# hpcaitech/SkyComputing

Measured on AMD Instinct MI355X. Metric: sec_per_iter_bert160_mnli_bsz32, lower is better.
Workload: dtype bf16; 1 GPU; model=bert-160L-H1024-A16, global_batch=32, seq_len=128, parallelism=pp1, microbatches=1, schedule=gpipe, allocate=even, num_pipeline_layers=483, hipgraph=True

## Files before the change

skycomputing_amd/ops/build.py:

```python

from __future__ import annotations

import glob
import hashlib
import json
import os
import subprocess
import sys

HIP_DIR = os.path.join(os.path.dirname(os.path.abspath(__file__)), "hip")
LIB = os.path.join(HIP_DIR, "libskyhip.so")
STAMP = os.path.join(HIP_DIR, ".build_stamp.json")

HIPCC = os.environ.get("HIPCC", "hipcc")
ARCH = os.environ.get("SKY_GFX_ARCH", "gfx950")
CFLAGS = [
    f"--offload-arch={ARCH}", "-O3", "-std=c++17", "-fPIC",
    "-fvisibility=hidden", "-Wall", "-Wno-unused-function",
]


def _source_hash(sources: list[str]) -> str:
    h = hashlib.sha256()
    for s in sorted(sources) + sorted(glob.glob(os.path.join(HIP_DIR, "*.h"))):
        with open(s, "rb") as f:
            h.update(f.read())
    h.update(" ".join(CFLAGS).encode())
    return h.hexdigest()


def build(force: bool = False, verbose: bool = True) -> str:
    sources = sorted(glob.glob(os.path.join(HIP_DIR, "*.hip")))
    if not sources:
        raise RuntimeError(f"no .hip sources under {HIP_DIR}")
    want = _source_hash(sources)
    if not force and os.path.isfile(LIB) and os.path.isfile(STAMP):
        try:
            with open(STAMP) as f:
                if json.load(f).get("hash") == want:
                    if verbose:
                        print(f"[skyhip] up to date: {LIB}")
                    return LIB
        except Exception:
            pass
    objs = []
    for src in sources:
        obj = src.replace(".hip", ".o")
        cmd = [HIPCC, *CFLAGS, "-x", "hip", "-c", src, "-o", obj]
        if verbose:
            print("[skyhip]", " ".join(cmd))
        subprocess.run(cmd, check=True)
        objs.append(obj)
# ... 15 lines not shown
```

skycomputing_amd/ops/hip/attention_bwd.hip:

```cpp

#include "attn_common.h"

template <bool HAS_MASK, bool DBIAS>
__global__ __launch_bounds__(256, 3) void attn_bwd1s_kernel(
    const ushort_t* __restrict__ qkv, const ushort_t* __restrict__ dout,
    const ushort_t* __restrict__ mask, const float* __restrict__ m_io,
    const float* __restrict__ l_io, ushort_t* __restrict__ pdT,
    ushort_t* __restrict__ dsT, ushort_t* __restrict__ dqkv, int B, int S,
    int h, float scale, float keep, uint64_t salt,
    const unsigned long long* __restrict__ state, float* __restrict__ dbscr) {
  extern __shared__ __attribute__((aligned(16))) char lds[];
  const int tid = threadIdx.x;
  const int l = tid & 63;
  const int w = tid >> 6;
  const int lm = l & 15;
  const int lg = l >> 4;
  const int QB = (S + 63) / 64;
  const int bh = blockIdx.x / QB;
  const int qb = blockIdx.x % QB;
  const int b = bh / h;
  const int hh = bh % h;
  const int ts = 3 * h * ATT_D;
  const int NT = (S + 15) / 16;
  const uint64_t seed = rng_seed(salt, state);
// ... 46 lines not shown
    float mrow[4], lrow[4], dot[4];
    uint64_t zs[4][2];
#pragma unroll
    for (int r = 0; r < 4; ++r) {
      const int row = qtok_base + lg * 4 + r;
      const int rr = row < S ? row : S - 1;
      mrow[r] = m_io[(size_t)bh * S + rr];
      lrow[r] = 1.f / l_io[(size_t)bh * S + rr];
      dot[r] = 0.f;
      zs[r][0] = zs[r][1] = 0;
      if (keep < 1.f) att_drop_hash(zs[r], seed, bh, S, row, lm);
    }
#pragma unroll
    for (int r = 0; r < 4; ++r) {
      const int row = qtok_base + lg * 4 + r;
#pragma unroll
      for (int kt = 0; kt < 8; ++kt) {
        if (kt >= NT) continue;
        const int col = kt * 16 + lm;
        const float p = att_prob(sacc[kt][r], scale, mval[kt], mrow[r],
                                 lrow[r], row < S && col < S);
        float dp = dacc[kt][r];
        if (keep < 1.f) dp = att_drop_keep(zs[r], kt, keep16) ? dp * inv_keep : 0.f;
        dot[r] += dp * p;
      }
    }
#pragma unroll
    for (int r = 0; r < 4; ++r) dot[r] = row16_sum(dot[r]);
#pragma unroll
    for (int kt = 0; kt < 8; ++kt) {
      if (kt >= NT) continue;
      const int col = kt * 16 + lm;
      ushort4_t ds4, pd4;
#pragma unroll
      for (int r = 0; r < 4; ++r) {
        const int row = qtok_base + lg * 4 + r;
        const float p = att_prob(sacc[kt][r], scale, mval[kt], mrow[r],
                                 lrow[r], row < S && col < S);
        float pd = p, dp = dacc[kt][r];
        if (keep < 1.f) {
          const bool kbit = att_drop_keep(zs[r], kt, keep16);
          pd = kbit ? p * inv_keep : 0.f;
          dp = kbit ? dp * inv_keep : 0.f;
        }
        const float ds = scale * p * (dp - dot[r]);
        const int rl = lg * 4 + r;
        *(ushort_t*)lds_at(lds, swz(32768 + w * 4096 + rl * 256 + col * 2, rl, 15)) =
            f32_to_bf16(ds);
        ds4[r] = f32_to_bf16(ds);
        pd4[r] = f32_to_bf16(pd);
      }
      if (col < S) {
        const size_t o = ((size_t)bh * S + col) * S + qtok_base + lg * 4;
        if (qtok_base + lg * 4 + 3 < S) {
          *(ushort4_t*)(dsT + o) = ds4;
          *(ushort4_t*)(pdT + o) = pd4;
        } else {
#pragma unroll
          for (int r = 0; r < 4; ++r)
            if (qtok_base + lg * 4 + r < S) {
              dsT[o + r] = ds4[r];
              pdT[o + r] = pd4[r];
            }
        }
      }
    }
  }
  __syncthreads();

  float cs[4] = {0.f, 0.f, 0.f, 0.f};
  if (active) {
    f32x4 qacc[4];
    att_zero(qacc);
#pragma unroll
    for (int ks = 0; ks < 4; ++ks) {
      if (ks * 32 >= S) break;
      bf16x8 asr = *(const bf16x8*)lds_at(
          lds, swz(32768 + w * 4096 + lm * 256 + (ks * 32 + lg * 8) * 2, lm, 15));
#pragma unroll
      for (int ct = 0; ct < 4; ++ct) {
        bf16x8 bkt = abf_tr_rows64(lds, 16384, ks * 32 + lg * 8, ct * 4, lm);
        qacc[ct] = __builtin_amdgcn_mfma_f32_16x16x32_bf16(asr, bkt, qacc[ct], 0, 0, 0);
      }
// ... 390 lines not shown
```

skycomputing_amd/ops/hip/attn_common.h:

```cpp
#pragma once

#include "common.h"

typedef const __attribute__((address_space(1))) unsigned int* att_gas;
typedef __attribute__((address_space(3))) unsigned int* att_las;

typedef __attribute__((ext_vector_type(8))) short bf16x8;
typedef __attribute__((ext_vector_type(4))) float f32x4;

#define ATT_SMAX 128
#define ATT_D 64

DEV void* lds_at(char* base, int byte) { return (void*)(base + byte); }

DEV int swz(int byte_addr, int row, int rmask) {
  return byte_addr ^ ((row & rmask) << 4);
}

typedef __attribute__((ext_vector_type(4))) short s16x4_a;
typedef __attribute__((address_space(3))) s16x4_a* abf_las4;

DEV bf16x8 abf_tr_rows64(const char* lds_base, int off, int r0, int cq0,
                         int s4) {
  s16x4_a v[2];
// ... 78 lines not shown
    int gtok = tok0 + tok;
    if (clamp && gtok >= S) gtok = S - 1;
    const int c16s = (u & 7) ^ (tok & 7);
    __builtin_amdgcn_global_load_lds(
        (att_gas)(src + (size_t)gtok * tstride + c16s * 8),
        (att_las)lds_at(lds, off + u * 16), 16, 0, 0);
  }
}

DEV float att_prob(float s, float scale, float mv, float m, float inv_l,
                   bool valid) {
  float p = __expf(s * scale + mv - m) * inv_l;
  if (!valid) p = 0.f;
  return p;
}

DEV void att_drop_hash(uint64_t (&z)[2], uint64_t seed, int bh, int S,
                       int row, int lm) {
  const uint64_t base = ((uint64_t)bh * S + row) * 16 + lm;
  z[0] = rng_hash(seed, base * 2);
  z[1] = rng_hash(seed, base * 2 + 1);
}
DEV bool att_drop_keep(const uint64_t (&z)[2], int kt, unsigned keep16) {
  const uint64_t zz = kt < 4 ? z[0] : z[1];
  return (unsigned)((zz >> (16 * (kt & 3))) & 0xFFFFu) < keep16;
}

DEV void att_store_rows16(ushort_t* __restrict__ dst, int rstride,
                          const f32x4 (&acc)[4], int row0, int S, int lm,
                          int lg) {
#pragma unroll
  for (int ct = 0; ct < 4; ++ct) {
#pragma unroll
    for (int r = 0; r < 4; ++r) {
      const int row = row0 + lg * 4 + r;
      if (row < S) dst[(size_t)row * rstride + ct * 16 + lm] = f32_to_bf16(acc[ct][r]);
    }
  }
}

DEV void att_store_rows16x2(ushort_t* __restrict__ d0,
                            ushort_t* __restrict__ d1, int rstride,
                            const f32x4 (&a0)[4], const f32x4 (&a1)[4],
                            int row0, int S, int lm, int lg) {
#pragma unroll
  for (int ct = 0; ct < 4; ++ct) {
#pragma unroll
    for (int r = 0; r < 4; ++r) {
      const int row = row0 + lg * 4 + r;
      const int c = ct * 16 + lm;
      if (row < S) {
        d0[(size_t)row * rstride + c] = f32_to_bf16(a0[ct][r]);
        d1[(size_t)row * rstride + c] = f32_to_bf16(a1[ct][r]);
      }
    }
  }
}

DEV void att_colsum_rows16(float (&cs)[4], const f32x4 (&acc)[4], int row0,
                           int S, int lg) {
#pragma unroll
  for (int ct = 0; ct < 4; ++ct) {
#pragma unroll
    for (int r = 0; r < 4; ++r)
      if (row0 + lg * 4 + r < S) cs[ct] += bf16_to_f32(f32_to_bf16(acc[ct][r]));
  }
}

DEV void att_colsum_wave(float (&cs)[4]) {
#pragma unroll
  for (int ct = 0; ct < 4; ++ct) {
    cs[ct] += __shfl_xor(cs[ct], 16, 64);
    cs[ct] += __shfl_xor(cs[ct], 32, 64);
  }
}

#define ATT_LAUNCH_HM(has_mask, KERNEL, grid, lds_bytes, stream, ...)         \
  do {                                                                        \
    if (has_mask) {                                                           \
      constexpr bool HM = true;                                               \
      hipLaunchKernelGGL(KERNEL, grid, dim3(256), lds_bytes, stream,          \
                         __VA_ARGS__);                                        \
    } else {                                                                  \
      constexpr bool HM = false;                                              \
      hipLaunchKernelGGL(KERNEL, grid, dim3(256), lds_bytes, stream,          \
                         __VA_ARGS__);                                        \
// ... 3 lines not shown
```

skycomputing_amd/ops/hip/common.h:

```cpp
#pragma once

#include <hip/hip_runtime.h>
#include <hip/hip_bf16.h>
#include <stdint.h>
#include <type_traits>

#define WAVE 64
#define DEV __device__ __forceinline__

typedef unsigned short ushort_t;
typedef __attribute__((ext_vector_type(2))) unsigned short ushort2_t;
typedef __attribute__((ext_vector_type(4))) unsigned short ushort4_t;
typedef __attribute__((ext_vector_type(8))) unsigned short ushort8_t;
typedef __attribute__((ext_vector_type(4))) float float4_t;

DEV float bf16_to_f32(ushort_t u) {
  union { unsigned int i; float f; } v;
  v.i = ((unsigned int)u) << 16;
  return v.f;
}

DEV ushort_t f32_to_bf16(float f) {
  union { unsigned int i; float f; } v;
  v.f = f;
  unsigned int lsb = (v.i >> 16) & 1u;
  v.i += 0x7fffu + lsb;
  return (ushort_t)(v.i >> 16);
}

enum { DT_F32 = 0, DT_BF16 = 1 };

template <int DT> struct Vec8;
template <> struct Vec8<DT_BF16> {
  static DEV void load(const void* p, int64_t i8, float f[8]) {
    ushort8_t v = ((const ushort8_t*)p)[i8];
#pragma unroll
    for (int j = 0; j < 8; ++j) f[j] = bf16_to_f32(v[j]);
  }
  static DEV void store(void* p, int64_t i8, const float f[8]) {
    ushort8_t v;
#pragma unroll
    for (int j = 0; j < 8; ++j) v[j] = f32_to_bf16(f[j]);
    ((ushort8_t*)p)[i8] = v;
  }
};
template <> struct Vec8<DT_F32> {
  static DEV void load(const void* p, int64_t i8, float f[8]) {
    float4_t a = ((const float4_t*)p)[i8 * 2];
    float4_t b = ((const float4_t*)p)[i8 * 2 + 1];
#pragma unroll
    for (int j = 0; j < 4; ++j) { f[j] = a[j]; f[4 + j] = b[j]; }
  }
  static DEV void store(void* p, int64_t i8, const float f[8]) {
    float4_t a, b;
#pragma unroll
    for (int j = 0; j < 4; ++j) { a[j] = f[j]; b[j] = f[4 + j]; }
    ((float4_t*)p)[i8 * 2] = a;
    ((float4_t*)p)[i8 * 2 + 1] = b;
  }
};

template <int DT> DEV float load_elem(const void* p, int64_t i);
template <> DEV float load_elem<DT_F32>(const void* p, int64_t i) {
  return ((const float*)p)[i];
}
template <> DEV float load_elem<DT_BF16>(const void* p, int64_t i) {
  return bf16_to_f32(((const ushort_t*)p)[i]);
}
template <int DT> DEV void store_elem(void* p, int64_t i, float v);
template <> DEV void store_elem<DT_F32>(void* p, int64_t i, float v) {
  ((float*)p)[i] = v;
}
template <> DEV void store_elem<DT_BF16>(void* p, int64_t i, float v) {
  ((ushort_t*)p)[i] = f32_to_bf16(v);
}

// ... 35 lines not shown
}

DEV uint64_t rng_seed(uint64_t salt, const unsigned long long* state) {
  return salt + (state ? *state : 0ull) * 0xD1B54A32D192ED03ull;
}

DEV float rng_uniform(uint64_t seed, uint64_t idx) {
  return (float)(rng_hash(seed, idx) >> 40) * 0x1.0p-24f;
}

DEV bool rng_keep16(uint64_t seed, uint64_t idx, unsigned keep16) {
  uint64_t z = rng_hash(seed, idx >> 2);
  return (unsigned)((z >> (16 * (idx & 3))) & 0xFFFFu) < keep16;
}

#define RNG_DROP8(seed, i8, keep16, inv_keep, v, bits)                        \
  do {                                                                        \
    const uint64_t z0_ = rng_hash(seed, (uint64_t)(i8) * 2);                  \
    const uint64_t z1_ = rng_hash(seed, (uint64_t)(i8) * 2 + 1);              \
    bits = 0;                                                                 \
    _Pragma("unroll") for (int j_ = 0; j_ < 8; ++j_) {                        \
      const uint64_t zz_ = j_ < 4 ? z0_ : z1_;                                \
      const bool kb_ =                                                        \
          (unsigned)((zz_ >> (16 * (j_ & 3))) & 0xFFFFu) < (keep16);          \
      bits |= (unsigned)kb_ << j_;                                            \
      (v)[j_] = kb_ ? (v)[j_] * (inv_keep) : 0.f;                             \
    }                                                                         \
  } while (0)

DEV unsigned keep_to_16(float keep) {
  return keep >= 1.f ? 0x20000u : (unsigned)(keep * 65536.f + 0.5f);
}

DEV float erf_fast(float x) {
  const float ax = fabsf(x);
  const float t = 1.f / fmaf(0.3275911f, ax, 1.f);
  const float p = t * fmaf(t, fmaf(t, fmaf(t, fmaf(t, 1.061405429f, -1.453152027f),
                                           1.421413741f), -0.284496736f),
                           0.254829592f);
  const float r = 1.f - p * __expf(-ax * ax);
  return copysignf(r, x);
}
DEV float gelu_f(float x) { return 0.5f * x * (1.f + erf_fast(x * 0.70710678118654752f)); }
DEV float gelu_grad_f(float x) {
  const float k = 0.70710678118654752f;
  const float c = 0.3989422804014327f;
  float cdf = 0.5f * (1.f + erf_fast(x * k));
  float pdf = c * __expf(-0.5f * x * x);
  return cdf + x * pdf;
}

void sky_launch_colsum_final(hipStream_t s, const float* scratch, void* out,
                             int64_t cols, int64_t nslabs, int dtout);

struct SkyFinishJob {
  uint64_t scratch;
  uint64_t out[3];
  int64_t nslabs;
  int64_t cols;
  int32_t nv;
  int32_t dtout;
};
constexpr int SKY_FINISH_MAX_JOBS = 4;

static inline void sky_finish_job_set(SkyFinishJob* job, uint64_t scratch,
                                      uint64_t o0, uint64_t o1, uint64_t o2,
                                      int64_t nslabs, int64_t cols, int nv,
                                      int dtout) {
  *job = SkyFinishJob{scratch, {o0, o1, o2}, nslabs, cols, nv, dtout};
}

constexpr int MAX_SLABS = 1024;

template <int MAXCH = 8, class F>
static inline void dispatch_tags(int dt, bool has_res, bool drop, int ch,
                                 F&& f) {
  using std::integral_constant;
  auto by_ch = [&](auto DT, auto HR, auto DR) {
    if (ch <= 2) f(DT, HR, DR, integral_constant<int, 2>{});
    else if (ch <= 4) f(DT, HR, DR, integral_constant<int, 4>{});
    else if constexpr (MAXCH >= 8) f(DT, HR, DR, integral_constant<int, 8>{});
// ... 15 lines not shown
```

skycomputing_amd/ops/hip/elementwise.hip:

```cpp

#include "common.h"


template <int DT>
__global__ __launch_bounds__(256) void bias_gelu_fwd_vec_kernel(
    const void* __restrict__ x, const void* __restrict__ b,
    void* __restrict__ y, int64_t n8, int64_t cols8) {
  for (int64_t i8 = (int64_t)blockIdx.x * 256 + threadIdx.x; i8 < n8;
       i8 += (int64_t)gridDim.x * 256) {
    float v[8], bv[8];
    Vec8<DT>::load(x, i8, v);
    Vec8<DT>::load(b, i8 % cols8, bv);
#pragma unroll
    for (int j = 0; j < 8; ++j) v[j] = gelu_f(v[j] + bv[j]);
    Vec8<DT>::store(y, i8, v);
  }
}

template <int DT>
__global__ __launch_bounds__(256) void bias_gelu_fwd_kernel(
    const void* __restrict__ x, const void* __restrict__ b,
    void* __restrict__ y, int64_t n, int64_t cols) {
  for (int64_t i = (int64_t)blockIdx.x * 256 + threadIdx.x; i < n;
       i += (int64_t)gridDim.x * 256) {
// ... 74 lines not shown
  float bv[8];
  if (HAS_B) Vec8<DT>::load(b, c8, bv);
  float s[8] = {0.f};
  for (int64_t r = r0; r < r1; ++r) {
    float v[8], d[8];
    Vec8<DT>::load(x, r * cols8 + c8, v);
    Vec8<DT>::load(dy, r * cols8 + c8, d);
#pragma unroll
    for (int j = 0; j < 8; ++j) {
      d[j] *= gelu_grad_f(HAS_B ? v[j] + bv[j] : v[j]);
      s[j] += d[j];
    }
    Vec8<DT>::store(dx, r * cols8 + c8, d);
  }
#pragma unroll
  for (int j = 0; j < 8; ++j) scratch[(slab * cols8 + c8) * 8 + j] = s[j];
}

template <int DT, bool HAS_B>
__global__ __launch_bounds__(256) void bias_gelu_bwd_cs_kernel(
    const void* __restrict__ dy, const void* __restrict__ x,
    const void* __restrict__ b, void* __restrict__ dx,
    float* __restrict__ scratch, int64_t rows, int64_t cols8,
    int64_t rows_per_slab) {
  const int64_t nwin = cols8 >> 8;
  const int64_t win = blockIdx.x % nwin;
  const int64_t slab = blockIdx.x / nwin;
  const int64_t c8 = win * 256 + threadIdx.x;
  const int64_t r0 = slab * rows_per_slab;
  const int64_t r1 = min(rows, r0 + rows_per_slab);
  float bv[8];
  if (HAS_B) Vec8<DT>::load(b, c8, bv);
  float s[8] = {0.f};
  for (int64_t r = r0; r < r1; ++r) {
    float v[8], d[8];
    Vec8<DT>::load(x, r * cols8 + c8, v);
    Vec8<DT>::load(dy, r * cols8 + c8, d);
#pragma unroll
    for (int j = 0; j < 8; ++j) {
      d[j] *= gelu_grad_f(HAS_B ? v[j] + bv[j] : v[j]);
      s[j] += d[j];
    }
    Vec8<DT>::store(dx, r * cols8 + c8, d);
  }
#pragma unroll
  for (int j = 0; j < 8; ++j) scratch[(slab * cols8 + c8) * 8 + j] = s[j];
}

template <int DT, int BLOCK>
__global__ __launch_bounds__(BLOCK) void colsum_part_kernel(
    const void* __restrict__ src, float* __restrict__ scratch, int64_t rows,
    int64_t cols8, int64_t rows_per_slab) {
  const int64_t c8 = (int64_t)blockIdx.x * BLOCK + threadIdx.x;
  if (c8 >= cols8) return;
  const int64_t slab = blockIdx.y;
  const int64_t r0 = slab * rows_per_slab;
  const int64_t r1 = min(rows, r0 + rows_per_slab);
  float s[8] = {0.f};
  for (int64_t r = r0; r < r1; ++r) {
    float v[8];
    Vec8<DT>::load(src, r * cols8 + c8, v);
#pragma unroll
    for (int j = 0; j < 8; ++j) s[j] += v[j];
  }
#pragma unroll
  for (int j = 0; j < 8; ++j) scratch[(slab * cols8 + c8) * 8 + j] = s[j];
}

template <int BLOCK, int DTOUT>
__global__ __launch_bounds__(1024) void colsum_final_kernel(
    const float* __restrict__ scratch, void* __restrict__ out, int64_t cols,
    int64_t nslabs) {
  __shared__ float lds[64][17];
  const int c = threadIdx.x & 15;
  const int g = threadIdx.x >> 4;
  const int64_t col = (int64_t)blockIdx.x * 16 + c;
// ... 359 lines not shown
```

skycomputing_amd/ops/hip/gemm2.hip:

```cpp

#include "common.h"

typedef __attribute__((ext_vector_type(8))) short bf16x8;
typedef __attribute__((ext_vector_type(4))) float f32x4;

#define G2_BM 256
#define G2_BN 256
#define G2_BK 64
#define G2_BLOCK 512
#define G2_LDS (128 * 1024)

typedef const __attribute__((address_space(1))) unsigned int* g2_gas;
typedef __attribute__((address_space(3))) unsigned int* g2_las;

DEV void g2_glds16(const void* g, void* l) {
  __builtin_amdgcn_global_load_lds((g2_gas)g, (g2_las)l, 16, 0, 0);
}

DEV int g2_swz(int byte_addr, int row) { return byte_addr ^ ((row & 7) << 4); }

enum { G2_EPI_NONE = 0, G2_EPI_BIAS = 1, G2_EPI_BIAS_GELU = 2 };

enum { G2_DIRECT = 0, G2_KMAJOR = 1 };

// ... 214 lines not shown
  }

  if (SPLIT) {
    float* out = Wk + (size_t)g * M * N;
#pragma unroll
    for (int i = 0; i < 8; ++i) {
      const int m = m0 + wr * 128 + i * 16 + lg * 4;
#pragma unroll
      for (int j = 0; j < 4; ++j) {
        const int n = n0 + wc * 64 + j * 16 + lm;
#pragma unroll
        for (int r = 0; r < 4; ++r)
          __builtin_nontemporal_store(acc[i][j][r],
                                      out + (size_t)(m + r) * N + n);
      }
    }
    return;
  }

  float bv[4];
  if (EPI != G2_EPI_NONE) {
#pragma unroll
    for (int j = 0; j < 4; ++j) {
      const int n = n0 + wc * 64 + j * 16 + lm;
      bv[j] = bias ? bf16_to_f32(bias[n]) : 0.f;
    }
  }
#pragma unroll
  for (int i = 0; i < 8; ++i) {
#pragma unroll
    for (int r = 0; r < 4; ++r) {
      const int m = m0 + wr * 128 + i * 16 + lg * 4 + r;
#pragma unroll
      for (int j = 0; j < 4; ++j) {
        const int n = n0 + wc * 64 + j * 16 + lm;
        float v = acc[i][j][r];
        if (EPI != G2_EPI_NONE) v += bv[j];
        if (EPI == G2_EPI_BIAS_GELU) {
          if (STORE_Z) Z[(size_t)m * ldc + n] = f32_to_bf16(v);
          v = gelu_f(v);
        }
        C[(size_t)m * ldc + n] = f32_to_bf16(v);
      }
    }
  }
}

template <int EPI, bool STORE_Z>
__global__ __launch_bounds__(256) void gemm2_reduce_kernel(
    const float* __restrict__ Wk, ushort_t* __restrict__ C,
    const ushort_t* __restrict__ bias, ushort_t* __restrict__ Z, long MN,
    int N, int ldc, int gsu) {
  const long i4 = ((long)blockIdx.x * 256 + threadIdx.x) * 4;
  if (i4 >= MN) return;
  f32x4 s = *(const f32x4*)(Wk + i4);
  for (int g = 1; g < gsu; ++g) {
    f32x4 p = *(const f32x4*)(Wk + (size_t)g * MN + i4);
#pragma unroll
    for (int r = 0; r < 4; ++r) s[r] += p[r];
  }
  const int m = (int)(i4 / N), n = (int)(i4 % N);
  ushort4_t o, zo;
#pragma unroll
  for (int r = 0; r < 4; ++r) {
    float v = s[r];
    if (EPI != G2_EPI_NONE) v += bf16_to_f32(bias[n + r]);
    if (EPI == G2_EPI_BIAS_GELU) {
      if (STORE_Z) zo[r] = f32_to_bf16(v);
      v = gelu_f(v);
    }
    o[r] = f32_to_bf16(v);
  }
  *(ushort4_t*)(C + (size_t)m * ldc + n) = o;
  if (EPI == G2_EPI_BIAS_GELU && STORE_Z) *(ushort4_t*)(Z + (size_t)m * ldc + n) = zo;
}

static int g2_set_lds(const void* f) {
  static const void* done[32];
  static int ndone = 0;
  for (int i = 0; i < ndone; ++i)
    if (done[i] == f) return 0;
  hipError_t e = hipFuncSetAttribute(
      f, hipFuncAttributeMaxDynamicSharedMemorySize, G2_LDS);
  if (e != hipSuccess) return (int)e;
  if (ndone < 32) done[ndone++] = f;
  return 0;
}

SKY_EXPORT int sky_gemm2(uint64_t stream, uint64_t A, uint64_t B, uint64_t C,
                         uint64_t bias, uint64_t Z, uint64_t Wk, int64_t M,
                         int64_t N, int64_t K, int64_t lda, int64_t ldb,
                         int64_t ldc, int transA, int transB, int epi,
                         int gsu) {
  if (M % G2_BM || N % G2_BN || K % G2_BK) return (int)hipErrorInvalidValue;
  if (gsu > 1 && (K % (gsu * G2_BK) || !Wk)) return (int)hipErrorInvalidValue;
  if (lda % 8 || ldb % 8 || ldc % 8) return (int)hipErrorInvalidValue;
  hipStream_t s = (hipStream_t)stream;
  const long ntiles = (M / G2_BM) * (N / G2_BN);
  dim3 grid((unsigned)(ntiles * (gsu > 1 ? gsu : 1)));
  const bool split = gsu > 1;
  const bool sz = Z != 0;
  int rc = 0;
#define G2K(AM, BM, EP, SZ, SP)                                                \
  do {                                                                         \
    rc = g2_set_lds((const void*)&gemm2_kernel<AM, BM, EP, SZ, SP>);           \
// ... 50 lines not shown
```

skycomputing_amd/ops/hip/layernorm.hip:

```cpp

#include "common.h"

#define LN_MAXCH 8


template <int CTRL, int ROW_MASK>
DEV float dpp_add(float v) {
  const int t = __builtin_amdgcn_update_dpp(0, __float_as_int(v), CTRL,
                                            ROW_MASK, 0xf, true);
  return v + __int_as_float(t);
}
DEV float wave_sum_dpp(float v) {
  v = dpp_add<0x111, 0xf>(v);
  v = dpp_add<0x112, 0xf>(v);
  v = dpp_add<0x114, 0xf>(v);
  v = dpp_add<0x118, 0xf>(v);
  v = dpp_add<0x142, 0xa>(v);
  v = dpp_add<0x143, 0xc>(v);
  return __int_as_float(__builtin_amdgcn_readlane(__float_as_int(v), 63));
}

struct LnDrop {
  uint64_t seed;
  unsigned keep16;
// ... 129 lines not shown
                                 uint64_t w, uint64_t b, uint64_t y,
                                 uint64_t mean, uint64_t rstd, int64_t rows,
                                 int64_t cols, float eps, int dt, float keep,
                                 uint64_t salt, uint64_t state) {
  hipStream_t s = (hipStream_t)stream;
  bool has_res = res != 0;
  bool drop = keep < 1.f;
  if (drop && !ln_fast_ok(cols)) return (int)hipErrorInvalidValue;
  if (ln_fast_ok(cols)) {
    unsigned grid = (unsigned)((rows + 3) / 4);
    if (grid > 8192u) grid = 8192u;
    dispatch_tags(dt, has_res, drop, ln_chunks(cols),
                  [&](auto DT, auto HR, auto DR, auto CH) {
      hipLaunchKernelGGL((ln_fwd_vec_kernel<DT, HR, DR, CH>), dim3(grid),
                         dim3(256), 0, s, (const void*)x, (const void*)res,
                         (const void*)w, (const void*)b, (void*)y,
                         (float*)mean, (float*)rstd, rows, cols, eps, keep,
                         salt, (const unsigned long long*)state);
    });
  } else {
    dim3 grid((unsigned)(rows < 4096 ? rows : 4096));
    dispatch_tags(dt, has_res, false, 0, [&](auto DT, auto HR, auto, auto) {
      hipLaunchKernelGGL((ln_fwd_kernel<DT, 256, HR>), grid, dim3(256), 0, s,
                         (const void*)x, (const void*)res, (const void*)w,
                         (const void*)b, (void*)y, (float*)mean, (float*)rstd,
                         rows, cols, eps);
    });
  }
  LAUNCH_CHECK();
  return 0;
}


template <int DT, bool HAS_RES, bool DROP, int CH, int NS>
__global__ __launch_bounds__(256) void ln_bwd_dx_cs_kernel(
    const void* __restrict__ dy, const void* __restrict__ x,
    const void* __restrict__ res, const void* __restrict__ w,
    const float* __restrict__ mean, const float* __restrict__ rstd,
    void* __restrict__ dx, void* __restrict__ dres,
    float* __restrict__ scratch, int64_t rows, int64_t cols, float keep,
    uint64_t salt, const unsigned long long* __restrict__ state) {
  const int lane = threadIdx.x & (WAVE - 1);
  const int wid = threadIdx.x / WAVE;
  const int64_t cols8 = cols / 8;
  const LnDrop drop(DROP, keep, salt, state);
  float xh[CH][8], dxh[CH][8];
  float sw[NS ? CH : 1][8], sb[NS ? CH : 1][8], sx[NS == 3 ? CH : 1][8];
  if constexpr (NS > 0) {
#pragma unroll
    for (int c = 0; c < CH; ++c)
#pragma unroll
      for (int j = 0; j < 8; ++j) {
        sw[c][j] = 0.f;
        sb[c][j] = 0.f;
        if constexpr (NS == 3) sx[c][j] = 0.f;
      }
  }
  unsigned kbits[CH];
  for (int64_t row = (int64_t)blockIdx.x * 4 + wid; row < rows;
       row += (int64_t)gridDim.x * 4) {
    const int64_t base8 = row * cols8;
    const float mu = mean[row], rs = rstd[row];
    float s1 = 0.f, s2 = 0.f;
#pragma unroll
    for (int c = 0; c < CH; ++c) {
      const int64_t i8 = (int64_t)c * WAVE + lane;
      if (i8 < cols8) {
// ... 9 lines not shown
          s2 += dxh[c][j] * xh[c][j];
          if constexpr (NS > 0) {
            sw[c][j] += dyv[j] * xh[c][j];
            sb[c][j] += dyv[j];
          }
        }
      }
    }
    s1 = wave_sum(s1) / (float)cols;
    s2 = wave_sum(s2) / (float)cols;
#pragma unroll
    for (int c = 0; c < CH; ++c) {
      const int64_t i8 = (int64_t)c * WAVE + lane;
      if (i8 < cols8) {
        float o[8];
#pragma unroll
        for (int j = 0; j < 8; ++j)
          o[j] = rs * (dxh[c][j] - s1 - xh[c][j] * s2);
        if (DROP && dres != nullptr) Vec8<DT>::store(dres, base8 + i8, o);
        if (DROP) {
#pragma unroll
          for (int j = 0; j < 8; ++j)
            o[j] = ((kbits[c] >> j) & 1u) ? o[j] * drop.inv_keep : 0.f;
        }
        if constexpr (NS == 3) {
#pragma unroll
          for (int j = 0; j < 8; ++j)
            sx[c][j] += DT == DT_BF16 ? bf16_to_f32(f32_to_bf16(o[j])) : o[j];
        }
        Vec8<DT>::store(dx, base8 + i8, o);
      }
    }
  }
  if constexpr (NS > 0) {
    __shared__ float mrg[NS][CH * 512];
    for (int i = threadIdx.x; i < NS * CH * 512; i += 256)
      (&mrg[0][0])[i] = 0.f;
    __syncthreads();
    for (int k = 0; k < 4; ++k) {
      if (wid == k) {
#pragma unroll
        for (int c = 0; c < CH; ++c) {
          const int64_t i8 = (int64_t)c * WAVE + lane;
          if (i8 < cols8) {
#pragma unroll
            for (int j = 0; j < 8; ++j) {
              mrg[0][i8 * 8 + j] += sw[c][j];
              mrg[1][i8 * 8 + j] += sb[c][j];
              if constexpr (NS == 3) mrg[2][i8 * 8 + j] += sx[c][j];
            }
          }
        }
      }
      __syncthreads();
    }
    float* base = scratch + (int64_t)blockIdx.x * NS * cols8 * 8;
    for (int i = threadIdx.x; i < cols8 * 8; i += 256) {
      base[i] = mrg[0][i];
      base[cols8 * 8 + i] = mrg[1][i];
      if constexpr (NS == 3) base[2 * cols8 * 8 + i] = mrg[2][i];
    }
  }
}

template <int DT, bool HAS_RES, bool DROP, int BLOCK>
__global__ __launch_bounds__(BLOCK) void ln_bwd_wb_part_kernel(
    const void* __restrict__ dy, const void* __restrict__ x,
// ... 109 lines not shown
    s2 = block_sum<BLOCK>(s2, lds) / (float)cols;
    for (int64_t c = threadIdx.x; c < cols; c += BLOCK) {
      float xv = load_elem<DT>(x, base + c);
      if (HAS_RES) xv += load_elem<DT>(res, base + c);
      float xhat = (xv - mu) * rs;
      float dxhat = load_elem<DT>(dy, base + c) * load_elem<DT>(w, c);
      store_elem<DT>(dx, base + c, rs * (dxhat - s1 - xhat * s2));
    }
  }
}

#define LN_XSUM_MAXCH 4

struct LnBwdArgs {
  hipStream_t s;
  uint64_t dy, x, res, w, mean, rstd, dx, dres, scratch;
  int64_t rows, cols;
  int dt;
  float keep;
  uint64_t salt, state;
};

template <int NS>
static int64_t ln_bwd_dx_launch(const LnBwdArgs& a) {
  unsigned gmax = 8192;
  if (NS > 0) {
    gmax = 512;
    if (const char* e = getenv("SKY_LN_CS_GRID")) gmax = (unsigned)atoi(e);
    if (gmax > (unsigned)MAX_SLABS) gmax = MAX_SLABS;
    if (gmax < 1) gmax = 1;
  }
  unsigned grid = (unsigned)((a.rows + 3) / 4);
  if (grid > gmax) grid = gmax;
  dispatch_tags<NS == 3 ? LN_XSUM_MAXCH : LN_MAXCH>(
      a.dt, a.res != 0, a.keep < 1.f, ln_chunks(a.cols),
      [&](auto DT, auto HR, auto DR, auto CH) {
        hipLaunchKernelGGL((ln_bwd_dx_cs_kernel<DT, HR, DR, CH, NS>),
                           dim3(grid), dim3(256), 0, a.s, (const void*)a.dy,
                           (const void*)a.x, (const void*)a.res,
                           (const void*)a.w, (const float*)a.mean,
                           (const float*)a.rstd, (void*)a.dx, (void*)a.dres,
                           (float*)a.scratch, a.rows, a.cols, a.keep, a.salt,
                           (const unsigned long long*)a.state);
      });
  return (int64_t)grid;
}

template <int NV>
static void ln_bwd_wb_final_launch(const LnBwdArgs& a, uint64_t dw,
                                   uint64_t db, uint64_t dxsum,
                                   int64_t nslabs) {
  auto launch = [&](auto kern) {
    hipLaunchKernelGGL(kern, dim3((unsigned)((a.cols + 15) / 16)), dim3(1024),
                       0, a.s, (const float*)a.scratch, (void*)dw, (void*)db,
                       (void*)dxsum, a.cols, nslabs);
  };
  if (a.dt == DT_BF16) launch(ln_bwd_wb_final_kernel<256, DT_BF16, NV>);
  else launch(ln_bwd_wb_final_kernel<256, DT_F32, NV>);
}

template <int NS>
static int ln_bwd_cs_launch(const LnBwdArgs& a, uint64_t dw, uint64_t db,
                            uint64_t dxsum, SkyFinishJob* job = nullptr) {
  const int64_t nslabs = ln_bwd_dx_launch<NS>(a);
  if (job)
    sky_finish_job_set(job, a.scratch, dw, db, dxsum, nslabs, a.cols, NS,
                       a.dt);
  else
    ln_bwd_wb_final_launch<NS>(a, dw, db, dxsum, nslabs);
  LAUNCH_CHECK();
  return 0;
}

SKY_EXPORT int sky_layernorm_bwd(uint64_t stream, uint64_t dy, uint64_t x,
                                 uint64_t res, uint64_t w, uint64_t mean,
                                 uint64_t rstd, uint64_t dx, uint64_t dw,
// ... 104 lines not shown
```

skycomputing_amd/ops/hip/sgd.hip:

```cpp

#include "common.h"

struct SgdDesc {
  uint64_t p, g, m, mom;
  int64_t n;
  int64_t pad;
};

template <int DT>
DEV void nt_load8(const void* p, int64_t i8, float f[8]);
template <>
DEV void nt_load8<DT_BF16>(const void* p, int64_t i8, float f[8]) {
  ushort8_t v = __builtin_nontemporal_load((const ushort8_t*)p + i8);
#pragma unroll
  for (int j = 0; j < 8; ++j) f[j] = bf16_to_f32(v[j]);
}
template <>
DEV void nt_load8<DT_F32>(const void* p, int64_t i8, float f[8]) {
  float4_t a = __builtin_nontemporal_load((const float4_t*)p + i8 * 2);
  float4_t b = __builtin_nontemporal_load((const float4_t*)p + i8 * 2 + 1);
#pragma unroll
  for (int j = 0; j < 4; ++j) { f[j] = a[j]; f[4 + j] = b[j]; }
}
template <int DT>
DEV void nt_store8(void* p, int64_t i8, const float f[8]);
template <>
DEV void nt_store8<DT_BF16>(void* p, int64_t i8, const float f[8]) {
  ushort8_t v;
#pragma unroll
  for (int j = 0; j < 8; ++j) v[j] = f32_to_bf16(f[j]);
  __builtin_nontemporal_store(v, (ushort8_t*)p + i8);
}
template <>
DEV void nt_store8<DT_F32>(void* p, int64_t i8, const float f[8]) {
  float4_t a, b;
#pragma unroll
  for (int j = 0; j < 4; ++j) { a[j] = f[j]; b[j] = f[4 + j]; }
  __builtin_nontemporal_store(a, (float4_t*)p + i8 * 2);
  __builtin_nontemporal_store(b, (float4_t*)p + i8 * 2 + 1);
}

template <int DT, int BLOCK, bool MASTER, bool MOM, int UNROLL = 2,
          bool NT = true>
__global__ __launch_bounds__(BLOCK) void sgd_kernel(
    const SgdDesc* __restrict__ descs, float lr, float momentum, float wd) {
  const SgdDesc d = descs[blockIdx.x];
  void* p = (void*)d.p;
  const void* g = (const void*)d.g;
  float* master = (float*)d.m;
  float* mbuf = (float*)d.mom;
  const int64_t n8 = d.n / 8;
  for (int64_t i8 = threadIdx.x; i8 < n8; i8 += UNROLL * BLOCK) {
#pragma unroll
    for (int u = 0; u < UNROLL; ++u) {
      const int64_t k8 = i8 + u * BLOCK;
      if (k8 >= n8) break;
      float gv[8], pv[8];
      if (NT) {
        nt_load8<DT>(g, k8, gv);
        if (MASTER) nt_load8<DT_F32>(master, k8, pv);
        else nt_load8<DT>(p, k8, pv);
      } else {
        Vec8<DT>::load(g, k8, gv);
        if (MASTER) Vec8<DT_F32>::load(master, k8, pv);
// ... 89 lines not shown
```

skycomputing_amd/ops/hiplib.py:

```python

from __future__ import annotations

import ctypes
import os

_LIB = None
_LIB_PATH = os.path.join(os.path.dirname(os.path.abspath(__file__)), "hip", "libskyhip.so")
_TRIED = False

_SIGNATURES: dict[str, list] = {}

FINISH_MAX_JOBS = 4

u64 = ctypes.c_uint64
i64 = ctypes.c_int64
i32 = ctypes.c_int32
f32 = ctypes.c_float
f64 = ctypes.c_double


class FinishJob(ctypes.Structure):

    _fields_ = [
        ("scratch", u64), ("out", u64 * 3), ("nslabs", i64), ("cols", i64),
        ("nv", i32), ("dtout", i32),
    ]


def _register_signatures(lib):
    sigs = {
        "sky_layernorm_fwd": [u64, u64, u64, u64, u64, u64, u64, u64, i64, i64, f32, i32, f32, u64, u64],
        "sky_layernorm_bwd": [u64, u64, u64, u64, u64, u64, u64, u64, u64, u64, u64, i64, i64, i32, f32, u64, u64, u64],
        "sky_layernorm_bwd_xsum": [u64, u64, u64, u64, u64, u64, u64, u64, u64, u64, u64, i64, i64, i32, f32, u64, u64, u64, u64],
        "sky_layernorm_bwd_xsum_ok": [i64],
        "sky_bias_gelu_fwd": [u64, u64, u64, u64, i64, i64, i32],
        "sky_bias_gelu_bwd": [u64, u64, u64, u64, u64, u64, u64, i64, i64, i32],
        "sky_masked_softmax_fwd": [u64, u64, u64, u64, i64, i64, i64, i64, f32, f32, u64, i32],
        "sky_masked_softmax_bwd": [u64, u64, u64, u64, i64, i64, i64, i64, f32, f32, u64, i32],
        "sky_embedding_fwd": [u64] * 12 + [i64, i64, i64, f32, i32],
        "sky_embedding_bwd": [u64] * 16 + [i64, i64, i32],
        "sky_sgd_step": [u64, u64, i64, f32, f32, f32, i32, i32],
        "sky_adamw_tick": [u64, u64, f64, f64],
        "sky_gradnorm_partials": [u64, u64, i64, u64, i32],
        "sky_gradnorm_finish": [u64, u64, i64, u64, f32],
        "sky_adamw_step": [u64, u64, i64, u64, f64, f64, f32, f32, i32, i32],
        "sky_detect_mem": [u64, u64],
        "sky_dropout_fwd": [u64, u64, u64, i64, f32, u64, u64, i32],
        "sky_dropout_bwd": [u64, u64, u64, i64, f32, u64, u64, i32],
        "sky_rng_tick": [u64, u64],
        "sky_colsum": [u64, u64, u64, u64, i64, i64, i32, i32],
        "sky_hblt_wgrad_bgrad": [u64, u64, u64, u64, u64, i64, i64, i64, i32],
        "sky_hblt_wgrad": [u64, u64, u64, u64, i64, i64, i64, i32],
        "sky_hblt_linear_gelu_aux": [u64, u64, u64, u64, u64, u64, i64, i64, i64, i32, i32],
        "sky_mfma_probe": [u64, u64, u64, u64],
        "sky_glds_probe": [u64, u64, u64, i32],
        "sky_gemm": [u64, u64, u64, u64, u64, u64, i64, i64, i64, i64, i64, i64, i32, i32, i32, i32, i32],
        "sky_gemm2": [u64, u64, u64, u64, u64, u64, u64, i64, i64, i64, i64, i64, i64, i32, i32, i32, i32],
        "sky_pack3": [u64, u64, u64, u64, u64, i64, i64, i64, i64, i32],
        "sky_attn_fwd": [u64, u64, u64, u64, u64, u64, i64, i64, i64, i64, f32, f32, u64, u64],
        "sky_attn_probs": [u64, u64, u64, u64, u64, u64, u64, i64, i64, i64, i64, f32, f32, u64, u64],
        "sky_attn_flash_fwd": [u64, u64, u64, u64, u64, u64, i64, i64, i64, i64, f32, f32, u64, u64],
        "sky_attn_bwd": [u64] * 9 + [i64, i64, i64, i64, f32, f32, u64, u64],
        "sky_attn_bwd_dbias": [u64] * 9 + [i64, i64, i64, i64, f32, f32, u64, u64, u64, u64, i32],
        "sky_attn_bwd_dbias_parts": [u64] * 9 + [i64, i64, i64, i64, f32, f32, u64, u64, u64, u64, i32, u64],
        "sky_layernorm_bwd_parts": [u64, u64, u64, u64, u64, u64, u64, u64, u64, u64, u64, i64, i64, i32, f32, u64, u64, u64, u64, u64],
        "sky_bias_gelu_bwd_parts": [u64, u64, u64, u64, u64, u64, u64, i64, i64, i32, u64],
        "sky_colsum_finish": [u64, u64, i32],
        "sky_attn_bwd_fused": [u64] * 7 + [i64, i64, i64, i64, f32, f32, u64, u64],
    }
    for name, argtypes in sigs.items():
        if hasattr(lib, name):
            fn = getattr(lib, name)
            fn.argtypes = argtypes
            fn.restype = ctypes.c_int
    return sigs


def lib():
    global _LIB, _TRIED
    if _LIB is None and not _TRIED:
        _TRIED = True
        if os.path.isfile(_LIB_PATH):
            _LIB = ctypes.CDLL(_LIB_PATH)
            _register_signatures(_LIB)
    return _LIB


def available() -> bool:
# ... 23 lines not shown
```

Baseline: 0.1014 sec/iter.

## Use hardware bf16 pack conversions, fast GELU math, and parallel LN-backward merge

Replaces the software round-to-nearest-even bf16 conversion with compiler `__bf16` conversions, adding paired and quad packing helpers used in attention, GEMM epilogues, elementwise and SGD stores. The goal is to let gfx950's packed f32-to-bf16 conversion instructions cut ALU work in epilogues. GELU backward now shares one exp between the cdf and pdf terms and uses a hardware reciprocal approximation, which may shift accuracy slightly. LayerNorm backward gains a per-wave LDS partial-sum merge that replaces the zeroed shared merge buffer. The diff also unrolls the bias-GELU backward row loop by two, and adds a probe kernel that checks rounding equivalence plus an env hook for extra compiler flags.

```diff
diff --git a/skycomputing_amd/ops/build.py b/skycomputing_amd/ops/build.py
--- a/skycomputing_amd/ops/build.py
+++ b/skycomputing_amd/ops/build.py
@@ -5,6 +5,7 @@
 import hashlib
 import json
 import os
+import shlex
 import subprocess
 import sys
 
@@ -18,6 +19,7 @@
     f"--offload-arch={ARCH}", "-O3", "-std=c++17", "-fPIC",
     "-fvisibility=hidden", "-Wall", "-Wno-unused-function",
 ]
+CFLAGS += shlex.split(os.environ.get("SKY_HIPCC_FLAGS", ""))
 
 
 def _source_hash(sources: list[str]) -> str:
diff --git a/skycomputing_amd/ops/hip/attention_bwd.hip b/skycomputing_amd/ops/hip/attention_bwd.hip
--- a/skycomputing_amd/ops/hip/attention_bwd.hip
+++ b/skycomputing_amd/ops/hip/attention_bwd.hip
@@ -102,6 +102,7 @@
       if (kt >= NT) continue;
       const int col = kt * 16 + lm;
       ushort4_t ds4, pd4;
+      float dsf[4], pdf[4];
 #pragma unroll
       for (int r = 0; r < 4; ++r) {
         const int row = qtok_base + lg * 4 + r;
@@ -114,11 +115,16 @@
           dp = kbit ? dp * inv_keep : 0.f;
         }
         const float ds = scale * p * (dp - dot[r]);
+        dsf[r] = ds;
+        pdf[r] = pd;
+      }
+      ds4 = f32x4_to_bf16x4(dsf[0], dsf[1], dsf[2], dsf[3]);
+      pd4 = f32x4_to_bf16x4(pdf[0], pdf[1], pdf[2], pdf[3]);
+#pragma unroll
+      for (int r = 0; r < 4; ++r) {
         const int rl = lg * 4 + r;
         *(ushort_t*)lds_at(lds, swz(32768 + w * 4096 + rl * 256 + col * 2, rl, 15)) =
-            f32_to_bf16(ds);
-        ds4[r] = f32_to_bf16(ds);
-        pd4[r] = f32_to_bf16(pd);
+            ds4[r];
       }
       if (col < S) {
         const size_t o = ((size_t)bh * S + col) * S + qtok_base + lg * 4;
diff --git a/skycomputing_amd/ops/hip/attn_common.h b/skycomputing_amd/ops/hip/attn_common.h
--- a/skycomputing_amd/ops/hip/attn_common.h
+++ b/skycomputing_amd/ops/hip/attn_common.h
@@ -134,9 +134,12 @@
 #pragma unroll
   for (int ct = 0; ct < 4; ++ct) {
 #pragma unroll
-    for (int r = 0; r < 4; ++r) {
+    for (int r = 0; r < 4; r += 2) {
       const int row = row0 + lg * 4 + r;
-      if (row < S) dst[(size_t)row * rstride + ct * 16 + lm] = f32_to_bf16(acc[ct][r]);
+      const unsigned int v2 = f32x2_to_bf16x2(acc[ct][r], acc[ct][r + 1]);
+      if (row < S) dst[(size_t)row * rstride + ct * 16 + lm] = (ushort_t)v2;
+      if (row + 1 < S)
+        dst[(size_t)(row + 1) * rstride + ct * 16 + lm] = (ushort_t)(v2 >> 16);
     }
   }
 }
@@ -148,12 +151,18 @@
 #pragma unroll
   for (int ct = 0; ct < 4; ++ct) {
 #pragma unroll
-    for (int r = 0; r < 4; ++r) {
+    for (int r = 0; r < 4; r += 2) {
       const int row = row0 + lg * 4 + r;
       const int c = ct * 16 + lm;
+      const unsigned int v0 = f32x2_to_bf16x2(a0[ct][r], a0[ct][r + 1]);
+      const unsigned int v1 = f32x2_to_bf16x2(a1[ct][r], a1[ct][r + 1]);
       if (row < S) {
-        d0[(size_t)row * rstride + c] = f32_to_bf16(a0[ct][r]);
-        d1[(size_t)row * rstride + c] = f32_to_bf16(a1[ct][r]);
+        d0[(size_t)row * rstride + c] = (ushort_t)v0;
+        d1[(size_t)row * rstride + c] = (ushort_t)v1;
+      }
+      if (row + 1 < S) {
+        d0[(size_t)(row + 1) * rstride + c] = (ushort_t)(v0 >> 16);
+        d1[(size_t)(row + 1) * rstride + c] = (ushort_t)(v1 >> 16);
       }
     }
   }
diff --git a/skycomputing_amd/ops/hip/bf16_round_probe.hip b/skycomputing_amd/ops/hip/bf16_round_probe.hip
--- /dev/null
+++ b/skycomputing_amd/ops/hip/bf16_round_probe.hip
@@ -0,0 +1,55 @@
+
+#include "common.h"
+
+DEV ushort_t bf16_round_formula(unsigned int i) {
+  const unsigned int lsb = (i >> 16) & 1u;
+  i += 0x7fffu + lsb;
+  return (ushort_t)(i >> 16);
+}
+
+DEV bool bf16_is_nan(ushort_t b) { return (b & 0x7fffu) > 0x7f80u; }
+
+constexpr unsigned PROBE_BLOCKS = 4096;
+
+__global__ __launch_bounds__(256) void bf16_round_probe_kernel(
+    unsigned long long* __restrict__ counts) {
+  const unsigned int t = blockIdx.x * 256u + threadIdx.x;
+  unsigned int bad = 0, nan_lost = 0, seen = 0;
+  for (unsigned int k = 0; k < 4096u; ++k) {
+    const unsigned int i = t + (k << 20);
+    const float f = __builtin_bit_cast(float, i);
+    const float g = __builtin_bit_cast(float, i * 2654435761u + 0x3f800001u);
+    const ushort_t ref = bf16_round_formula(i);
+    const ushort_t sc = f32_to_bf16(f);
+    const ushort_t lo = (ushort_t)f32x2_to_bf16x2(f, g);
+    const ushort_t hi = (ushort_t)(f32x2_to_bf16x2(g, f) >> 16);
+    if ((i & 0x7fffffffu) > 0x7f800000u) {
+      if (!bf16_is_nan(sc) || !bf16_is_nan(lo) || !bf16_is_nan(hi)) ++nan_lost;
+    } else {
+      if (sc != ref || lo != ref || hi != ref) ++bad;
+    }
+    ++seen;
+  }
+  for (int off = 32; off > 0; off >>= 1) {
+    bad += __shfl_xor(bad, off, 64);
+    nan_lost += __shfl_xor(nan_lost, off, 64);
+    seen += __shfl_xor(seen, off, 64);
+  }
+  if ((threadIdx.x & (WAVE - 1)) == 0) {
+    if (bad) atomicAdd(&counts[0], (unsigned long long)bad);
+    if (nan_lost) atomicAdd(&counts[1], (unsigned long long)nan_lost);
+    atomicAdd(&counts[2], (unsigned long long)seen);
+  }
+}
+
+SKY_EXPORT int sky_probe_bf16_round(uint64_t stream, uint64_t counts) {
+  if (counts == 0) return (int)hipErrorInvalidValue;
+  hipStream_t s = (hipStream_t)stream;
+  hipError_t e =
+      hipMemsetAsync((void*)counts, 0, 3 * sizeof(unsigned long long), s);
+  if (e != hipSuccess) return (int)e;
+  hipLaunchKernelGGL(bf16_round_probe_kernel, dim3(PROBE_BLOCKS), dim3(256), 0,
+                     s, (unsigned long long*)counts);
+  LAUNCH_CHECK();
+  return 0;
+}
diff --git a/skycomputing_amd/ops/hip/common.h b/skycomputing_amd/ops/hip/common.h
--- a/skycomputing_amd/ops/hip/common.h
+++ b/skycomputing_amd/ops/hip/common.h
@@ -20,12 +20,24 @@
   return v.f;
 }
 
+typedef __attribute__((ext_vector_type(2))) float float2_t;
+typedef __attribute__((ext_vector_type(2))) __bf16 bf16x2_t;
+typedef __attribute__((ext_vector_type(2))) unsigned int uint2_t;
+typedef __attribute__((ext_vector_type(4))) unsigned int uint4_t;
+
 DEV ushort_t f32_to_bf16(float f) {
-  union { unsigned int i; float f; } v;
-  v.f = f;
-  unsigned int lsb = (v.i >> 16) & 1u;
-  v.i += 0x7fffu + lsb;
-  return (ushort_t)(v.i >> 16);
+  return __builtin_bit_cast(ushort_t, (__bf16)f);
+}
+
+DEV unsigned int f32x2_to_bf16x2(float lo, float hi) {
+  const float2_t v = {lo, hi};
+  return __builtin_bit_cast(unsigned int,
+                            __builtin_convertvector(v, bf16x2_t));
+}
+
+DEV ushort4_t f32x4_to_bf16x4(float a, float b, float c, float d) {
+  const uint2_t v = {f32x2_to_bf16x2(a, b), f32x2_to_bf16x2(c, d)};
+  return __builtin_bit_cast(ushort4_t, v);
 }
 
 enum { DT_F32 = 0, DT_BF16 = 1 };
@@ -38,10 +50,10 @@
     for (int j = 0; j < 8; ++j) f[j] = bf16_to_f32(v[j]);
   }
   static DEV void store(void* p, int64_t i8, const float f[8]) {
-    ushort8_t v;
-#pragma unroll
-    for (int j = 0; j < 8; ++j) v[j] = f32_to_bf16(f[j]);
-    ((ushort8_t*)p)[i8] = v;
+    uint4_t v;
+#pragma unroll
+    for (int j = 0; j < 4; ++j) v[j] = f32x2_to_bf16x2(f[2 * j], f[2 * j + 1]);
+    ((uint4_t*)p)[i8] = v;
   }
 };
 template <> struct Vec8<DT_F32> {
@@ -143,21 +155,36 @@
   return keep >= 1.f ? 0x20000u : (unsigned)(keep * 65536.f + 0.5f);
 }
 
-DEV float erf_fast(float x) {
+
+DEV float erf_fast_e(float x, float e) {
   const float ax = fabsf(x);
+#ifdef SKY_GELU_IEEE_MATH
   const float t = 1.f / fmaf(0.3275911f, ax, 1.f);
+#else
+  const float t = __builtin_amdgcn_rcpf(fmaf(0.3275911f, ax, 1.f));
+#endif
   const float p = t * fmaf(t, fmaf(t, fmaf(t, fmaf(t, 1.061405429f, -1.453152027f),
                                            1.421413741f), -0.284496736f),
                            0.254829592f);
-  const float r = 1.f - p * __expf(-ax * ax);
+  const float r = 1.f - p * e;
   return copysignf(r, x);
+}
+DEV float erf_fast(float x) {
+  const float ax = fabsf(x);
+  return erf_fast_e(x, __expf(-ax * ax));
 }
 DEV float gelu_f(float x) { return 0.5f * x * (1.f + erf_fast(x * 0.70710678118654752f)); }
 DEV float gelu_grad_f(float x) {
   const float k = 0.70710678118654752f;
   const float c = 0.3989422804014327f;
+#ifdef SKY_GELU_IEEE_MATH
   float cdf = 0.5f * (1.f + erf_fast(x * k));
   float pdf = c * __expf(-0.5f * x * x);
+#else
+  const float e = __expf(-0.5f * x * x);
+  float cdf = 0.5f * (1.f + erf_fast_e(x * k, e));
+  float pdf = c * e;
+#endif
   return cdf + x * pdf;
 }
 
diff --git a/skycomputing_amd/ops/hip/elementwise.hip b/skycomputing_amd/ops/hip/elementwise.hip
--- a/skycomputing_amd/ops/hip/elementwise.hip
+++ b/skycomputing_amd/ops/hip/elementwise.hip
@@ -130,16 +130,29 @@
   float bv[8];
   if (HAS_B) Vec8<DT>::load(b, c8, bv);
   float s[8] = {0.f};
-  for (int64_t r = r0; r < r1; ++r) {
-    float v[8], d[8];
-    Vec8<DT>::load(x, r * cols8 + c8, v);
-    Vec8<DT>::load(dy, r * cols8 + c8, d);
+  auto row = [&](int64_t r, const float (&v)[8], float (&d)[8]) {
 #pragma unroll
     for (int j = 0; j < 8; ++j) {
       d[j] *= gelu_grad_f(HAS_B ? v[j] + bv[j] : v[j]);
       s[j] += d[j];
     }
     Vec8<DT>::store(dx, r * cols8 + c8, d);
+  };
+  int64_t r = r0;
+  for (; r + 1 < r1; r += 2) {
+    float va[8], da[8], vb[8], db[8];
+    Vec8<DT>::load(x, r * cols8 + c8, va);
+    Vec8<DT>::load(dy, r * cols8 + c8, da);
+    Vec8<DT>::load(x, (r + 1) * cols8 + c8, vb);
+    Vec8<DT>::load(dy, (r + 1) * cols8 + c8, db);
+    row(r, va, da);
+    row(r + 1, vb, db);
+  }
+  if (r < r1) {
+    float v[8], d[8];
+    Vec8<DT>::load(x, r * cols8 + c8, v);
+    Vec8<DT>::load(dy, r * cols8 + c8, d);
+    row(r, v, d);
   }
 #pragma unroll
   for (int j = 0; j < 8; ++j) scratch[(slab * cols8 + c8) * 8 + j] = s[j];
diff --git a/skycomputing_amd/ops/hip/gemm2.hip b/skycomputing_amd/ops/hip/gemm2.hip
--- a/skycomputing_amd/ops/hip/gemm2.hip
+++ b/skycomputing_amd/ops/hip/gemm2.hip
@@ -270,15 +270,22 @@
     for (int r = 0; r < 4; ++r) {
       const int m = m0 + wr * 128 + i * 16 + lg * 4 + r;
 #pragma unroll
-      for (int j = 0; j < 4; ++j) {
+      for (int j = 0; j < 4; j += 2) {
         const int n = n0 + wc * 64 + j * 16 + lm;
-        float v = acc[i][j][r];
-        if (EPI != G2_EPI_NONE) v += bv[j];
+        float v0 = acc[i][j][r], v1 = acc[i][j + 1][r];
+        if (EPI != G2_EPI_NONE) { v0 += bv[j]; v1 += bv[j + 1]; }
         if (EPI == G2_EPI_BIAS_GELU) {
-          if (STORE_Z) Z[(size_t)m * ldc + n] = f32_to_bf16(v);
-          v = gelu_f(v);
+          if (STORE_Z) {
+            const unsigned int z2 = f32x2_to_bf16x2(v0, v1);
+            Z[(size_t)m * ldc + n] = (ushort_t)z2;
+            Z[(size_t)m * ldc + n + 16] = (ushort_t)(z2 >> 16);
+          }
+          v0 = gelu_f(v0);
+          v1 = gelu_f(v1);
         }
-        C[(size_t)m * ldc + n] = f32_to_bf16(v);
+        const unsigned int c2 = f32x2_to_bf16x2(v0, v1);
+        C[(size_t)m * ldc + n] = (ushort_t)c2;
+        C[(size_t)m * ldc + n + 16] = (ushort_t)(c2 >> 16);
       }
     }
   }
@@ -298,17 +305,19 @@
     for (int r = 0; r < 4; ++r) s[r] += p[r];
   }
   const int m = (int)(i4 / N), n = (int)(i4 % N);
+  float v[4];
   ushort4_t o, zo;
 #pragma unroll
   for (int r = 0; r < 4; ++r) {
-    float v = s[r];
-    if (EPI != G2_EPI_NONE) v += bf16_to_f32(bias[n + r]);
-    if (EPI == G2_EPI_BIAS_GELU) {
-      if (STORE_Z) zo[r] = f32_to_bf16(v);
-      v = gelu_f(v);
-    }
-    o[r] = f32_to_bf16(v);
-  }
+    v[r] = s[r];
+    if (EPI != G2_EPI_NONE) v[r] += bf16_to_f32(bias[n + r]);
+  }
+  if (EPI == G2_EPI_BIAS_GELU) {
+    if (STORE_Z) zo = f32x4_to_bf16x4(v[0], v[1], v[2], v[3]);
+#pragma unroll
+    for (int r = 0; r < 4; ++r) v[r] = gelu_f(v[r]);
+  }
+  o = f32x4_to_bf16x4(v[0], v[1], v[2], v[3]);
   *(ushort4_t*)(C + (size_t)m * ldc + n) = o;
   if (EPI == G2_EPI_BIAS_GELU && STORE_Z) *(ushort4_t*)(Z + (size_t)m * ldc + n) = zo;
 }
diff --git a/skycomputing_amd/ops/hip/layernorm.hip b/skycomputing_amd/ops/hip/layernorm.hip
--- a/skycomputing_amd/ops/hip/layernorm.hip
+++ b/skycomputing_amd/ops/hip/layernorm.hip
@@ -185,7 +185,8 @@
 }
 
 
-template <int DT, bool HAS_RES, bool DROP, int CH, int NS>
+#define LN_PMERGE_OK(DROP, CH, NS) ((CH) <= 2 && (NS) > 0 && (DROP))
+template <int DT, bool HAS_RES, bool DROP, int CH, int NS, bool PMERGE = false>
 __global__ __launch_bounds__(256) void ln_bwd_dx_cs_kernel(
     const void* __restrict__ dy, const void* __restrict__ x,
     const void* __restrict__ res, const void* __restrict__ w,
@@ -261,7 +262,46 @@
       }
     }
   }
-  if constexpr (NS > 0) {
+  if constexpr (NS > 0 && PMERGE) {
+    static_assert(LN_PMERGE_OK(DROP, CH, NS), "see LN_PMERGE_OK");
+    __shared__ __attribute__((aligned(16))) float part[4][NS][CH * 512];
+#pragma unroll
+    for (int c = 0; c < CH; ++c)
+#pragma unroll
+      for (int j = 0; j < 8; ++j) {
+        asm volatile("" : "+v"(sw[c][j]), "+v"(sb[c][j]));
+        if constexpr (NS == 3) asm volatile("" : "+v"(sx[c][j]));
+      }
+#pragma unroll
+    for (int c = 0; c < CH; ++c) {
+      const int64_t i8 = (int64_t)c * WAVE + lane;
+      if (i8 < cols8) {
+        float4_t* pw = (float4_t*)&part[wid][0][i8 * 8];
+        float4_t* pb = (float4_t*)&part[wid][1][i8 * 8];
+        pw[0] = float4_t{sw[c][0], sw[c][1], sw[c][2], sw[c][3]};
+        pw[1] = float4_t{sw[c][4], sw[c][5], sw[c][6], sw[c][7]};
+        pb[0] = float4_t{sb[c][0], sb[c][1], sb[c][2], sb[c][3]};
+        pb[1] = float4_t{sb[c][4], sb[c][5], sb[c][6], sb[c][7]};
+        if constexpr (NS == 3) {
+          float4_t* px = (float4_t*)&part[wid][2][i8 * 8];
+          px[0] = float4_t{sx[c][0], sx[c][1], sx[c][2], sx[c][3]};
+          px[1] = float4_t{sx[c][4], sx[c][5], sx[c][6], sx[c][7]};
+        }
+      }
+    }
+    __syncthreads();
+    float* base = scratch + (int64_t)blockIdx.x * NS * cols8 * 8;
+    const int n4 = (int)(cols8 * 2);
+    for (int i4 = threadIdx.x; i4 < n4; i4 += 256) {
+#pragma unroll
+      for (int v = 0; v < NS; ++v) {
+        float4_t a = {0.f, 0.f, 0.f, 0.f};
+#pragma unroll
+        for (int k = 0; k < 4; ++k) a += *(const float4_t*)&part[k][v][i4 * 4];
+        *(float4_t*)(base + (int64_t)v * cols8 * 8 + (int64_t)i4 * 4) = a;
+      }
+    }
+  } else if constexpr (NS > 0) {
     __shared__ float mrg[NS][CH * 512];
     for (int i = threadIdx.x; i < NS * CH * 512; i += 256)
       (&mrg[0][0])[i] = 0.f;
@@ -437,16 +477,28 @@
   }
   unsigned grid = (unsigned)((a.rows + 3) / 4);
   if (grid > gmax) grid = gmax;
+  [[maybe_unused]] const bool serial =
+      NS > 0 &&
+      (getenv("SKY_LN_MERGE_SERIAL") != nullptr || (a.scratch & 15) != 0);
   dispatch_tags<NS == 3 ? LN_XSUM_MAXCH : LN_MAXCH>(
       a.dt, a.res != 0, a.keep < 1.f, ln_chunks(a.cols),
       [&](auto DT, auto HR, auto DR, auto CH) {
-        hipLaunchKernelGGL((ln_bwd_dx_cs_kernel<DT, HR, DR, CH, NS>),
-                           dim3(grid), dim3(256), 0, a.s, (const void*)a.dy,
-                           (const void*)a.x, (const void*)a.res,
-                           (const void*)a.w, (const float*)a.mean,
-                           (const float*)a.rstd, (void*)a.dx, (void*)a.dres,
-                           (float*)a.scratch, a.rows, a.cols, a.keep, a.salt,
-                           (const unsigned long long*)a.state);
+        auto launch = [&](auto kern) {
+          hipLaunchKernelGGL(kern, dim3(grid), dim3(256), 0, a.s,
+                             (const void*)a.dy, (const void*)a.x,
+                             (const void*)a.res, (const void*)a.w,
+                             (const float*)a.mean, (const float*)a.rstd,
+                             (void*)a.dx, (void*)a.dres, (float*)a.scratch,
+                             a.rows, a.cols, a.keep, a.salt,
+                             (const unsigned long long*)a.state);
+        };
+        if constexpr (LN_PMERGE_OK(DR, CH, NS)) {
+          if (!serial) {
+            launch(ln_bwd_dx_cs_kernel<DT, HR, DR, CH, NS, true>);
+            return;
+          }
+        }
+        launch(ln_bwd_dx_cs_kernel<DT, HR, DR, CH, NS, false>);
       });
   return (int64_t)grid;
 }
diff --git a/skycomputing_amd/ops/hip/sgd.hip b/skycomputing_amd/ops/hip/sgd.hip
--- a/skycomputing_amd/ops/hip/sgd.hip
+++ b/skycomputing_amd/ops/hip/sgd.hip
@@ -26,10 +26,10 @@
 DEV void nt_store8(void* p, int64_t i8, const float f[8]);
 template <>
 DEV void nt_store8<DT_BF16>(void* p, int64_t i8, const float f[8]) {
-  ushort8_t v;
+  uint4_t v;
 #pragma unroll
-  for (int j = 0; j < 8; ++j) v[j] = f32_to_bf16(f[j]);
-  __builtin_nontemporal_store(v, (ushort8_t*)p + i8);
+  for (int j = 0; j < 4; ++j) v[j] = f32x2_to_bf16x2(f[2 * j], f[2 * j + 1]);
+  __builtin_nontemporal_store(v, (uint4_t*)p + i8);
 }
 template <>
 DEV void nt_store8<DT_F32>(void* p, int64_t i8, const float f[8]) {
diff --git a/skycomputing_amd/ops/hiplib.py b/skycomputing_amd/ops/hiplib.py
--- a/skycomputing_amd/ops/hiplib.py
+++ b/skycomputing_amd/ops/hiplib.py
@@ -54,6 +54,7 @@
         "sky_hblt_linear_gelu_aux": [u64, u64, u64, u64, u64, u64, i64, i64, i64, i32, i32],
         "sky_mfma_probe": [u64, u64, u64, u64],
         "sky_glds_probe": [u64, u64, u64, i32],
+        "sky_probe_bf16_round": [u64, u64],
         "sky_gemm": [u64, u64, u64, u64, u64, u64, i64, i64, i64, i64, i64, i64, i32, i32, i32, i32, i32],
         "sky_gemm2": [u64, u64, u64, u64, u64, u64, u64, i64, i64, i64, i64, i64, i64, i32, i32, i32, i32],
         "sky_pack3": [u64, u64, u64, u64, u64, i64, i64, i64, i64, i32],
```

Result: faster. 0.09939 sec/iter, median of 6 (-2.0%).
